# matt-suncy/symbols-from-video

Measured on AMD Instinct MI355X. Metric: frames/sec (enc+binarise+dec fwd+bwd), batch 256x256, 1/2/4/8 MI355X, higher is better.
Workload: dtype bf16; 1 GPU; percep_RBVAE fused train step (batch gather from the HBM-resident latent table + fwd+bwd+losses+Adam), item [16,2,8,4,32,32] per GPU = 256 frames/step/GPU (latents of 256x256 frames), latent 32, 4-layer LSTMs, dropout on; parallelism=dp1, graph=True, dist_world_size=1, schedule=one HIP graph per step, devices_visible=1, graphs_captured=1, launcher=torch.distributed.run or self-spawned ranks

## Files before the change

include/rbvae_dbg_variants.h:

```cpp
#ifndef RBVAE_DBG_VARIANTS_H
#define RBVAE_DBG_VARIANTS_H
#ifdef __cplusplus
extern "C" {
#endif
int rbvae_dbg_wgrad_gemm_variant(int v);

int rbvae_dbg_deconv_last_variant(int v);

#ifdef __cplusplus
}
#endif
#endif
```

include/rbvae_hip.h:

```cpp
#ifndef RBVAE_HIP_H
#define RBVAE_HIP_H

#include <stddef.h>
#include <stdint.h>

#ifdef __cplusplus
extern "C" {
#endif

#define RBVAE_OK 0
#define RBVAE_E_INVALID (-1)
#define RBVAE_E_LAUNCH (-2)
#define RBVAE_E_UNSUPPORTED (-3)

#define RBVAE_F32 0
#define RBVAE_BF16 1

int rbvae_version(void);
int rbvae_counter_add(unsigned long long* counter, unsigned long long inc, void* stream);
const char* rbvae_last_error(void);

int rbvae_binarize_kl_fwd(const float* h, const float* U, float* y_soft, float* z, float* kl_mean,
                          int rows, int L, float tau, float noise_ratio, float noise_eps, int hard,
                          float kl_p, float kl_eps, int kl_clamp, unsigned long long seed,
// ... 19 lines not shown
                       float* dx1, float* dx2, long dstride1, long dstride2, int accumulate, void* stream);
int rbvae_paircos_fwd(const float* x1, const float* x2, long stride1, long stride2, int rows, int L, int label,
                      float margin, float eps, float* out_mean, void* stream);
int rbvae_paircos_bwd(const float* x1, const float* x2, long stride1, long stride2, int rows, int L, int label,
                      float margin, float eps, float scale, const float* gscale_dev, float* dx1, float* dx2, long dstride1,
                      long dstride2, void* stream);
int rbvae_contrast_term_fwd(const float* h0, const float* h1, int B, int T, int L, float* out, void* stream);
int rbvae_contrast_term_bwd(const float* h0, const float* h1, int B, int T, int L, float scale,
                            const float* gscale_dev, float* dh0, float* dh1, void* stream);
int rbvae_contrast_term_nparts(int B, int T);
int rbvae_contrast_term_fused(const float* h0, const float* h1, int B, int T, int L, float scale,
                              const float* gscale_dev, float* parts, float* dh0, float* dh1, void* stream);
int rbvae_triplet_fwd(const float* a, const float* p, const float* n, long sa, long sp, long sn, int rows, int L,
                      float margin, float eps, int swap, float* out_mean, void* stream);
int rbvae_triplet_bwd(const float* a, const float* p, const float* n, long sa, long sp, long sn, int rows, int L,
                      float margin, float eps, int swap, float scale, const float* gscale_dev,
                      float* da, float* dp, float* dn, long dsa, long dsp, long dsn, int accumulate, void* stream);
int rbvae_triplet_term_fwd(const float* h0, const float* h1, int B, int T, int L, float margin, float* out,
                           void* stream);
int rbvae_triplet_term_bwd(const float* h0, const float* h1, int B, int T, int L, float margin, float scale,
                           const float* gscale_dev, float* dh0, float* dh1, void* stream);

size_t rbvae_mse_ws_floats(long n);
int rbvae_mse_fwd(const float* a, const float* b, long n, float* out_mean, float* ws, void* stream);
int rbvae_mse_bwd(const float* a, const float* b, long n, float scale, const float* gscale_dev, float* da,
                  void* stream);

int rbvae_gather_gemm(int dtype, const void* A, const void* W, void* Out, const float* bias, const void* gate,
                      const void* mask, const void* addend, const void* zero_page, int Nimg, int IH, int IW, int TH, int TW, int sa,
                      int OH, int OW, int so, int Kc, int Nout, int lda, int ldo, int taps_total, int nclass,
                      const int* class_desc, int relu, int drop_mode, float drop_p, float scale,
                      unsigned long long seed, const unsigned long long* seed_dev, float* colsum_ws,
                      void* stream);

int rbvae_conv3x3s2_halo_ok(int dtype, int Nimg, int IH, int IW, int Kc, int Nout);
int rbvae_conv3x3s2_halo_colsum_rows(int Nimg, int IH, int IW);
int rbvae_conv3x3s2_halo(int dtype, const void* A, const void* W, void* Out, const float* bias, const void* gate, const void* mask,
                         int Nimg, int IH, int IW, int Kc, int Nout, int lda, int ldo, int relu, int drop_mode, float drop_p,
                         float scale, unsigned long long seed, const unsigned long long* seed_dev, float* colsum_ws, void* stream);

int rbvae_fc_gemm_ok(int dtype, int M, int K, int N, int lda, int ldo);
int rbvae_fc_gemm(int dtype, const void* A, const void* W, void* Out, const float* bias, float* colsum_ws, int M, int K,
                  int N, int lda, int ldo, void* stream);

int rbvae_conv_gather_index(int* idx, int Nimg, int IH, int IW, int OH, int OW, int KH, int KW, int stride,
                            int pad, void* stream);
int rbvae_wgrad_gemm(int dtype, const void* Dy, const void* In, float* dW_slabs, const int* idx,
                     const void* zero_page, int P, int in_rows, int Co, int Ci, int ldy, int ldi, int taps, int ksplit,
                     void* stream);

int rbvae_wgrad3x3s2_halo_ok(int dtype, int Nimg, int OH, int OW, int Ca, int Cb);
int rbvae_wgrad3x3s2_halo_blocks(int Nimg, int OH, int OW);
int rbvae_wgrad3x3s2_halo(int dtype, const void* S, const void* G, float* dW_slabs, const void* zero_page, int Nimg, int OH,
                          int OW, int Ca, int Cb, int lds, int ldg, int ksplit, void* stream);

int rbvae_wgrad3x3s2_row_ok(int dtype, int Nimg, int OH, int OW, int Ca, int Cb);
int rbvae_wgrad3x3s2_row_blocks(int Nimg, int OH, int OW);
int rbvae_wgrad3x3s2_row(int dtype, const void* S, const void* G, float* dW_slabs, const void* zero_page, int Nimg, int OH,
                         int OW, int Ca, int Cb, int lds, int ldg, int ksplit, void* stream);

int rbvae_pack3(int dtype, const float* in, void* out, int d0, int d1, int d2, long s0, long s1, long s2,
                void* stream);
int rbvae_permute_reduce(const float* in, int nslab, long slab_stride, float* out, int d0, int d1, int d2, long s0,
                         long s1, long s2, float scale, int accumulate, void* stream);
int rbvae_cast_pad(int dtype, const float* in, void* out, int rows, int L, int Lpad, void* stream);
int rbvae_reduce_rows(const float* ws, int rows, int C, float* out, float scale, int accumulate, void* stream);
// ... 365 lines not shown
```

symbols-from-video_amd/build.py:

```python
import concurrent.futures
import os
import subprocess
import sys

HERE = os.path.dirname(os.path.abspath(__file__))
CSRC = os.path.join(HERE, "csrc")
OBJ = os.path.join(HERE, "build")
LIB = os.path.join(HERE, "librbvae_hip.so")
DBG_LIB = os.path.join(HERE, "librbvae_dbg.so")
DEBUG_LIB = os.path.join(HERE, "librbvae_hip_debug.so")
DBG_SOURCES = ("dbg.hip",)
HIPCC = os.environ.get("HIPCC", "/opt/rocm/bin/hipcc")
FLAGS = ["--offload-arch=gfx950", "-O3", "-fPIC", "-std=c++17", "-Wall", "-Wno-unused-function"]


def sources():
    return sorted(f for f in os.listdir(CSRC) if f.endswith(".hip"))


def _stale(target, deps):
    if not os.path.exists(target):
        return True
    t = os.path.getmtime(target)
    return any(os.path.getmtime(d) > t for d in deps)


def _compile(src, extra=(), suffix=""):
    obj = os.path.join(OBJ, src[:-4] + suffix + ".o")
    headers = [os.path.join(CSRC, f) for f in os.listdir(CSRC) if f.endswith(".h")]
    headers.append(os.path.join(os.path.dirname(HERE), "include", "rbvae_hip.h"))
    if _stale(obj, [os.path.join(CSRC, src)] + headers):
        cmd = [HIPCC] + FLAGS + list(extra) + ["-c", os.path.join(CSRC, src), "-o", obj]
        r = subprocess.run(cmd, capture_output=True, text=True)
        if r.returncode != 0:
            raise RuntimeError(f"hipcc failed on {src}:\n{r.stdout}\n{r.stderr}")
        if src in ISA_CHECKED and not extra:
            try:
                _check_asm_reads(src)
            except Exception:
                os.remove(obj)
                raise
        return obj, True
    return obj, False


ISA_CHECKED = {
    "wgrad_gemm.hip": ("_ZN5rbvae12wgrad_gemm_k", ("ds_read_b64_tr_b16",)),
    "gather_gemm.hip": ("_ZN5rbvae13gather_gemm_k", ("ds_read_b128",)),
    "conv_halo.hip": ("_ZN5rbvae11conv_halo_k", ("ds_read_b128",)),
    "conv_halo_ws.hip": ("_ZN5rbvae14conv_halo_ws_k", ("ds_read_b128",)),
    "deconv_halo.hip": ("_ZN5rbvae13deconv_halo_k", ("ds_read_b128",)),
    "wgrad_halo.hip": ("_ZN5rbvae12wgrad_halo_k", ("ds_read_b64_tr_b16",)),
    "wgrad_row.hip": ("_ZN5rbvae11wgrad_row_k", ("ds_read_b64_tr_b16",)),
    "conv_s2.hip": ("_ZN5rbvae9conv_s2_k", ("ds_read_b128",)),
    "upconv.hip": ("_ZN5rbvae13upconv_halo_k", ("ds_read_b128",)),
    "conv_first.hip": (("_ZN5rbvae13wgrad_first_k", "_ZN5rbvae18wgrad_first_wide_k"), ("ds_read_b64_tr_b16",)),
    "deconv_last_bwd.hip": ("_ZN5rbvae21deconv_last_fwd_bwd_k", ("ds_read_b128",)),
}


ASM_VMEM_LOADS = {"conv_halo.hip": "global_load_dwordx4", "deconv_halo.hip": "global_load_dwordx4",
                  "conv_halo_ws.hip": "buffer_load_dwordx4", "upconv.hip": "global_load_dwordx4"}


def _check_asm_reads(src):
    import importlib.util
    spec = importlib.util.spec_from_file_location("rbvae_isa_check", os.path.join(HERE, "isa_check.py"))
    mod = importlib.util.module_from_spec(spec)
    spec.loader.exec_module(mod)
    asm = os.path.join(OBJ, src[:-4] + ".s")
    cmd = [HIPCC] + FLAGS + ["-S", "--cuda-device-only", os.path.join(CSRC, src), "-o", asm]
    r = subprocess.run(cmd, capture_output=True, text=True)
    if r.returncode != 0:
        raise RuntimeError(f"hipcc -S failed on {src}:\n{r.stderr}")
    prefixes, ops = ISA_CHECKED[src]
    bad = []
    for prefix in ((prefixes,) if isinstance(prefixes, str) else prefixes):
        bad += mod.tr_asm_hazards(open(asm).read(), prefix, ops)
        if src in ASM_VMEM_LOADS:
            bad += mod.asm_vmem_load_hazards(open(asm).read(), prefix, ASM_VMEM_LOADS[src])
    if bad:
        raise RuntimeError(src + " ISA check failed (fragment register touched before its wait):\n" + "\n".join(bad[:20]))


def build(verbose=False):
    os.makedirs(OBJ, exist_ok=True)
    with concurrent.futures.ThreadPoolExecutor(max_workers=min(8, os.cpu_count() or 2)) as ex:
        res = list(ex.map(_compile, sources()))
    objs = [o for (o, _), src in zip(res, sources()) if src not in DBG_SOURCES]
    dbg_objs = [o for (o, _), src in zip(res, sources()) if src in DBG_SOURCES]

    def link(target, objects, extra=()):
        if _stale(target, objects) or any(c for _, c in res):
            cmd = [HIPCC, "--offload-arch=gfx950", "-shared", "-fPIC", "-o", target] + objects + list(extra)
            r = subprocess.run(cmd, capture_output=True, text=True)
            if r.returncode != 0:
                raise RuntimeError(f"link failed:\n{r.stdout}\n{r.stderr}")
            if verbose:
                print("built", target)

    link(LIB, objs)
    link(DBG_LIB, dbg_objs, ["-L" + HERE, "-lrbvae_hip", "-Wl,-rpath,$ORIGIN"])
    if os.environ.get("RBVAE_DEBUG") == "1":
        stamped = ["-DGG_STAMPS=1", "-DWG_STAMPS=1"]
        with concurrent.futures.ThreadPoolExecutor(max_workers=min(8, os.cpu_count() or 2)) as ex:
            dres = list(ex.map(lambda s_: _compile(s_, stamped, ".dbg"), [s_ for s_ in sources() if s_ not in DBG_SOURCES]))
        link(DEBUG_LIB, [o for o, _ in dres])
    return LIB


if __name__ == "__main__":
    build(verbose=True)
    sys.exit(0)
# ... 1 lines not shown
```

symbols-from-video_amd/csrc/dbg.hip:

```cpp
#include "mma.h"

namespace rbvae {

__global__ void dbg_mfma_bf16_k(const bf16_t* A, const bf16_t* B, float* D) {
    const int l = threadIdx.x, m = l & 15, g = l >> 4;
    bf16x8_t a, b;
    for (int j = 0; j < 8; ++j) {
        a[j] = (short)A[m * 32 + 8 * g + j];
        b[j] = (short)B[(8 * g + j) * 16 + m];
    }
    f32x4_t acc = {0.f, 0.f, 0.f, 0.f};
    acc = __builtin_amdgcn_mfma_f32_16x16x32_bf16(a, b, acc, 0, 0, 0);
    for (int r = 0; r < 4; ++r) D[(4 * g + r) * 16 + m] = acc[r];
}
__global__ void dbg_mfma_f32_k(const float* A, const float* B, float* D) {
    const int l = threadIdx.x, m = l & 15, g = l >> 4;
    f32x4_t acc = {0.f, 0.f, 0.f, 0.f};
    acc = __builtin_amdgcn_mfma_f32_16x16x4f32(A[m * 4 + g], B[g * 16 + m], acc, 0, 0, 0);
    for (int r = 0; r < 4; ++r) D[(4 * g + r) * 16 + m] = acc[r];
}
__global__ void dbg_glds_k(const unsigned* src, const int* lane_src_chunk, unsigned* out) {
    __shared__ __attribute__((aligned(16))) unsigned lds[256];
    const int l = threadIdx.x;
    glds16(src + 4 * lane_src_chunk[l], lds);
// ... 35 lines not shown
                       (bf16_t*)out);
    RBVAE_CHECK_LAUNCH("dbg_tr16");
    return RBVAE_OK;
}
}

namespace rbvae { extern int ch_variant; }
extern "C" int rbvae_dbg_conv_halo_variant(int v) {
    const int old = rbvae::ch_variant;
    rbvae::ch_variant = v;
    return old;
}

namespace rbvae { extern int lstm_unit_threads; }
extern "C" int rbvae_dbg_lstm_unit_threads(int v) {
    const int old = rbvae::lstm_unit_threads;
    rbvae::lstm_unit_threads = v;
    return old;
}

namespace rbvae { extern int wgrad_gemm_variant; }
extern "C" int rbvae_dbg_wgrad_gemm_variant(int v) {
    const int old = rbvae::wgrad_gemm_variant;
    rbvae::wgrad_gemm_variant = v;
    return old;
}

namespace rbvae { extern int deconv_last_variant; }
extern "C" int rbvae_dbg_deconv_last_variant(int v) {
    const int old = rbvae::deconv_last_variant;
    rbvae::deconv_last_variant = v;
    return old;
}
```

symbols-from-video_amd/csrc/gather_gemm.hip:

```cpp
#include "epilogue.h"
#include <stdlib.h>
#include <type_traits>

namespace rbvae {

struct TapClass {
    int ntaps;
    int oh0, ow0;
    signed char widx[16];
    signed char dh[16], dw[16];
};

struct GgArgs {
    const unsigned char* A;
    const unsigned char* W;
    unsigned char* Out;
    const float* bias;
    const unsigned char* gate;
    const unsigned char* mask;
    const unsigned char* addend;
    const unsigned char* zero;
    int Nimg, IH, IW;
    int TH, TW;
    int sa;
// ... 266 lines not shown
        int cbuf = 0;
        read_half(lds0, 0, fa0, fb0);
        const bool late = WAVES == 8 && w >= 4 && p.dephase;
        for (int s = 0; s + 1 < nsteps; ++s) {
            const unsigned lcur = lds0 + cbuf * STAGE;
            cbuf = (cbuf + 1 == GG_NS) ? 0 : cbuf + 1;
            read_half(lcur, 1, fa1, fb1);
            landed(Younger{}, fa0, fb0);
            __builtin_amdgcn_sched_barrier(0);
            mma_half(fa0, fb0);
            __builtin_amdgcn_sched_barrier(0);
            landed(None{}, fa1, fb1);
            if (GG_NS > 2 && nsteps - s - 2 >= GG_NS - 2) wait_vm_lgkm_barrier<(GG_NS > 2 ? GG_NS - 2 : 0) * LOADS>();
            else wait_vm_lgkm_barrier<0>();
            if (!late && s + GG_NS < nsteps) stage_next();
            read_half(lds0 + cbuf * STAGE, 0, fa0, fb0);
            __builtin_amdgcn_sched_barrier(0);
            mma_half(fa1, fb1);
            __builtin_amdgcn_sched_barrier(0);
            if (late && s + GG_NS < nsteps) stage_next();
        }
        {
            const unsigned lcur = lds0 + cbuf * STAGE;
            read_half(lcur, 1, fa1, fb1);
            landed(Younger{}, fa0, fb0);
            __builtin_amdgcn_sched_barrier(0);
            mma_half(fa0, fb0);
            __builtin_amdgcn_sched_barrier(0);
            landed(None{}, fa1, fb1);
            __builtin_amdgcn_sched_barrier(0);
            mma_half(fa1, fb1);
        }
    }
    GG_STAMP(3);
    __syncthreads();

    constexpr int CPR = BN / EC;
    constexpr int RL = THREADS / CPR;
    constexpr int ITERS = BM / RL;
    constexpr bool PREFETCH = GG_PREFETCH && ITERS <= 8;
    constexpr bool PF_LATE = GG_PREFETCH == 2;
    const int sch = tid % CPR, rl = tid / CPR;
    const int scol = n0 + sch * EC;
    int orow_[ITERS];
    u32x4_t gv[PREFETCH ? ITERS : 1], av[PREFETCH ? ITERS : 1];
#pragma unroll
    for (int it = 0; it < ITERS; ++it) {
        const int o = s_orow[it * RL + rl];
        orow_[it] = scol < p.Nout ? o : -1;
        if constexpr (PREFETCH && !PF_LATE) {
            const size_t off = ((size_t)(orow_[it] < 0 ? 0 : orow_[it]) * p.ldo + (orow_[it] < 0 ? 0 : scol)) * ES;
            if (p.gate) gv[it] = *(const u32x4_t*)(p.gate + off);
            if (p.addend) av[it] = *(const u32x4_t*)(p.addend + off);
        }
    }

    unsigned char* tile = smem;
#pragma unroll
    for (int nt = 0; nt < NTW; ++nt) {
        const int cb = (wc * NTW + nt) * 16 + 4 * fg;
#if GG_BIAS_LDS
        const float4 b4 = *(const float4*)(s_bias + cb);
        const float bz[4] = {b4.x, b4.y, b4.z, b4.w};
#else
        float bz[4] = {0.f, 0.f, 0.f, 0.f};
        if (p.bias && n0 + cb < p.Nout) {
            const float4 b4 = *(const float4*)(p.bias + n0 + cb);
            bz[0] = b4.x; bz[1] = b4.y; bz[2] = b4.z; bz[3] = b4.w;
        }
        (void)s_bias;
#endif
#pragma unroll
        for (int mt = 0; mt < MT; ++mt) {
            const int row = (wr * MT + mt) * 16 + fi;
            float v[4];
#pragma unroll
            for (int r = 0; r < 4; ++r) v[r] = epi_act(acc[mt][nt][r], bz[r], p.relu, p.scale);
            epi_stage<T>(tile + row * PITCH + cb * ES, v[0], v[1], v[2], v[3]);
        }
    }
    if constexpr (PREFETCH && PF_LATE) {
        if (p.gate) {
#pragma unroll
            for (int it = 0; it < ITERS; ++it) {
                const size_t off = ((size_t)(orow_[it] < 0 ? 0 : orow_[it]) * p.ldo + (orow_[it] < 0 ? 0 : scol)) * ES;
                gv[it] = *(const u32x4_t*)(p.gate + off);
            }
        }
    }
    __syncthreads();
    GG_STAMP(4);

    float csum[EC];
#pragma unroll
    for (int e = 0; e < EC; ++e) csum[e] = 0.f;
    DropKey dkey{0u, 0u};
    if (p.drop_mode == 1) dkey = epi_drop_key(p.seed, p.seed_dev);
#pragma unroll
    for (int it = 0; it < ITERS; ++it) {
        const int row = it * RL + rl;
        const int orow = orow_[it];
        if (orow >= 0) {
            const int col = scol;
            u32x4_t val = *(const u32x4_t*)(tile + row * PITCH + sch * 16);
            T* ev = (T*)&val;
            if (p.drop_mode == 1) {
                const unsigned run = drop_run(dkey, (unsigned long long)orow * p.Nout + col);
                if constexpr (sizeof(T) == 2) drop_chunk_zero_b16<EC>(run, p.drop_thresh >> 16, (unsigned*)&val);
                else drop_chunk_zero_f32<EC>(run, p.drop_thresh >> 16, (float*)&val);
            } else if (p.drop_mode == 2) {
                const unsigned char* mk = p.mask + (size_t)orow * p.Nout + col;
#pragma unroll
                for (int e = 0; e < EC; ++e)
                    if (!mk[e]) ev[e] = 0;
            }
            if (p.addend) {
                u32x4_t a4;
                if constexpr (PREFETCH && !PF_LATE) a4 = av[it];
                else a4 = *(const u32x4_t*)(p.addend + ((size_t)orow * p.ldo + col) * ES);
                const T* ae = (const T*)&a4;
#pragma unroll
                for (int e = 0; e < EC; ++e) Elem<T>::store(ev + e, Elem<T>::load(ev + e) + Elem<T>::load(ae + e));
            }
            if (p.gate) {
                u32x4_t g4;
                if constexpr (PREFETCH) g4 = gv[it];
                else g4 = *(const u32x4_t*)(p.gate + ((size_t)orow * p.ldo + col) * ES);
#pragma unroll
                for (int e = 0; e < EC; ++e)
                    if (!elem_pos<T>((const unsigned char*)&g4, e)) ev[e] = 0;
            }
            *(u32x4_t*)(p.Out + ((size_t)orow * p.ldo + col) * ES) = val;
            if (p.colsum_ws) {
#pragma unroll
                for (int e = 0; e < EC; ++e) csum[e] += Elem<T>::load(ev + e);
            }
        }
    }
    GG_STAMP(5);
    if (p.colsum_ws) {
        lds_barrier();
        float* red = (float*)smem;
#pragma unroll
        for (int e = 0; e < EC; ++e) red[rl * BN + sch * EC + e] = csum[e];
        lds_barrier();
        if (tid < BN && n0 + tid < p.Nout) {
            float t = 0.f;
#pragma unroll
            for (int k = 0; k < RL; ++k) t += red[k * BN + tid];
            p.colsum_ws[((size_t)bz * gridDim.x + bx) * p.Nout + n0 + tid] = t;
        }
    }
#if GG_STAMPS
    if (p.stamps) {
        asm volatile("s_waitcnt vmcnt(0)" ::: "memory");
        GG_STAMP(6);
    }
#endif
}

template <typename T, int NT, int WAVES, int NS, int OCC = 1, int BM = GG_BM>
static int launch_gg(const GgArgs& a, hipStream_t st) {
    constexpr int BN = NT * 32;
    constexpr int ES = sizeof(T);
    const int Mc = a.Nimg * a.TH * a.TW;
    const size_t ring = (size_t)NS * (BM * 128 + BN * 128);
    const size_t tile = (size_t)BM * (BN * ES + 16);
    const size_t lds = (ring > tile ? ring : tile) + BM * sizeof(int) + 64 * sizeof(int) + BN * sizeof(float);
    static bool attr_set = false;
    if (!attr_set) {
        hipFuncSetAttribute((const void*)gather_gemm_k<T, NT, WAVES, NS, OCC, BM>, hipFuncAttributeMaxDynamicSharedMemorySize,
                            (int)lds);
        attr_set = true;
    }
    dim3 grid(cdiv(Mc, BM), cdiv(a.Nout, BN), a.nclass);
    hipLaunchKernelGGL((gather_gemm_k<T, NT, WAVES, NS, OCC, BM>), grid, dim3(WAVES * 64), lds, st, a);
    RBVAE_CHECK_LAUNCH("gather_gemm");
    return RBVAE_OK;
}

#ifndef GG_RING64
#define GG_RING64 6
#endif
#ifndef GG_WAVES64
#define GG_WAVES64 4
#endif

template <typename T>
static int dispatch_gg(const GgArgs& a, hipStream_t st, int max_steps) {
    const long blocks = (long)cdiv(a.Nimg * a.TH * a.TW, GG_BM) * cdiv(a.Nout, a.Nout > 64 ? 128 : 64) * a.nclass;
    constexpr int force = 0;
    constexpr int dbg = 0;
    int ns = max_steps <= 2 ? 1 : (blocks > 256 ? 2 : 3);
    if (force) ns = force;
    if (ns == 3 && blocks > 128 && max_steps >= 8) ns = 4;
    if (a.Nout <= 64 && blocks <= 128 && max_steps >= 16 && sizeof(T) == 2 && !a.colsum_ws && !a.xcd_order)
        return launch_gg<T, 2, GG_WAVES64, GG_RING64, 1, 64>(a, st);
    if (a.Nout <= 64) return ns == 1 ? launch_gg<T, 2, 4, 1>(a, st) : launch_gg<T, 2, 4, 2>(a, st);
    constexpr int small = 2;
    if (ns == 3 && !force && !dbg && small) {
        constexpr int sq = 1;
        if (sq && small >= 2 && blocks <= 64 && !a.colsum_ws && !a.xcd_order && sizeof(T) == 2)
            return launch_gg<T, 2, GG_WAVES64, GG_RING64, 1, 64>(a, st);
        if (small >= 2 && blocks <= 64) return launch_gg<T, 1, 4, 3>(a, st);
        if (blocks <= 128) return launch_gg<T, 2, 4, 3>(a, st);
    }
    constexpr int one = 1;
    if (ns == 1 && one >= 1 && blocks > 512) return launch_gg<T, 2, 4, 1, 4>(a, st);
    if (ns == 1 && one >= 2 && blocks <= 64) return launch_gg<T, 1, 4, 1>(a, st);
    if (ns == 1) return launch_gg<T, 4, 4, 1>(a, st);
    if (ns >= 2 && (dbg == 5 || dbg == 6)) return dbg == 5 ? launch_gg<T, 2, 4, 3>(a, st) : launch_gg<T, 2, 4, 2>(a, st);
    if (ns == 2) return launch_gg<T, 4, 8, 2>(a, st);
    if (dbg == 4) return launch_gg<T, 4, 4, 3>(a, st);
    if (ns >= 4) return launch_gg<T, 4, 8, 4>(a, st);
    return launch_gg<T, 4, 8, 3>(a, st);
}

}

using namespace rbvae;

static unsigned long long* g_gg_stamps = nullptr;
#if GG_STAMPS
extern "C" int rbvae_dbg_gg_stamps(unsigned long long* buf, void* stream) {
    (void)stream;
    g_gg_stamps = buf;
    return RBVAE_OK;
}
#endif

extern "C" int rbvae_gather_gemm(int dtype, const void* A, const void* W, void* Out, const float* bias,
                                 const void* gate, const void* mask, const void* addend, const void* zero_page, int Nimg, int IH,
                                 int IW, int TH, int TW, int sa, int OH, int OW, int so, int Kc, int Nout, int lda,
                                 int ldo, int taps_total, int nclass, const int* class_desc, int relu,
                                 int drop_mode, float drop_p, float scale, unsigned long long seed,
                                 const unsigned long long* seed_dev, float* colsum_ws, void* stream) {
    RBVAE_CHECK_ARG(A && W && Out && zero_page && class_desc, "gather_gemm: null pointer");
    RBVAE_CHECK_ARG(dtype == RBVAE_F32 || dtype == RBVAE_BF16, "gather_gemm: dtype %d", dtype);
    const int ES = dtype == RBVAE_F32 ? 4 : 2;
    const int KE = 128 / ES;
    RBVAE_CHECK_ARG(Kc > 0 && Kc % KE == 0, "gather_gemm: Kc=%d must be a multiple of %d", Kc, KE);
    RBVAE_CHECK_ARG(Nout > 0 && Nout % 8 == 0, "gather_gemm: Nout=%d must be a multiple of 8", Nout);
    RBVAE_CHECK_ARG(lda >= Kc && (lda * ES) % 16 == 0 && ldo >= Nout && (ldo * ES) % 16 == 0,
                    "gather_gemm: leading dimensions lda=%d ldo=%d", lda, ldo);
    RBVAE_CHECK_ARG(nclass >= 1 && nclass <= 4, "gather_gemm: nclass=%d", nclass);
    RBVAE_CHECK_ARG(Nimg > 0 && IH > 0 && IW > 0 && TH > 0 && TW > 0 && OH > 0 && OW > 0, "gather_gemm: bad grid");
// ... 4 lines not shown
    GgArgs a;
    if (const int e = epi_drop_args("gather_gemm", drop_mode, mask, drop_p, &a.drop_thresh)) return e;
    a.A = (const unsigned char*)A; a.W = (const unsigned char*)W; a.Out = (unsigned char*)Out; a.bias = bias;
    a.gate = (const unsigned char*)gate; a.mask = (const unsigned char*)mask; a.addend = (const unsigned char*)addend;
    a.zero = (const unsigned char*)zero_page;
    a.Nimg = Nimg; a.IH = IH; a.IW = IW; a.TH = TH; a.TW = TW; a.sa = sa; a.OH = OH; a.OW = OW; a.so = so;
    a.Kc = Kc; a.Nout = Nout; a.lda = lda; a.ldo = ldo; a.taps_total = taps_total;
    a.relu = relu; a.drop_mode = drop_mode; a.scale = scale; a.seed = seed; a.seed_dev = seed_dev; a.colsum_ws = colsum_ws;
    a.nclass = nclass;
    constexpr int dephase = 1;
    a.dephase = dephase;
    constexpr int xcd = 0;
    a.xcd_order = xcd && cdiv(Nimg * TH * TW, GG_BM) % 8 == 0 && (nclass > 1 || cdiv(Nout, Nout > 64 ? 128 : 64) > 1);
    a.stamps = g_gg_stamps;
    auto log2_or_neg = [](int v) { int s = 0; while ((1 << s) < v) ++s; return (1 << s) == v ? s : -1; };
    a.sh_thw = log2_or_neg(TH * TW);
    a.sh_tw = log2_or_neg(TW);
    const int* d = class_desc;
    for (int c = 0; c < nclass; ++c) {
        TapClass& t = a.cls[c];
        t.ntaps = d[0]; t.oh0 = d[1]; t.ow0 = d[2];
        RBVAE_CHECK_ARG(t.ntaps >= 1 && t.ntaps <= 16, "gather_gemm: class %d has %d taps", c, t.ntaps);
        d += 3;
        for (int j = 0; j < t.ntaps; ++j) {
            RBVAE_CHECK_ARG(d[0] >= 0 && d[0] < taps_total, "gather_gemm: tap index %d outside [0,%d)", d[0], taps_total);
            t.widx[j] = (signed char)d[0]; t.dh[j] = (signed char)d[1]; t.dw[j] = (signed char)d[2];
            d += 3;
        }
    }
    hipStream_t st = (hipStream_t)stream;
    int max_taps = 0;
    for (int c = 0; c < nclass; ++c) max_taps = a.cls[c].ntaps > max_taps ? a.cls[c].ntaps : max_taps;
    const int max_steps = max_taps * (Kc / KE);
    return dtype == RBVAE_F32 ? dispatch_gg<float>(a, st, max_steps) : dispatch_gg<bf16_t>(a, st, max_steps);
}
```

Before: 588,700 frames/s.

## Add patch-reuse gather GEMM kernel for stride-2 3x3 convs sharing A tiles across taps

Adds a new gather_patch_k kernel for bf16 stride-2 single-class tap sets. Taps are grouped by input parity plane, so one staged A tile is reused across taps whose offsets differ only by a row or column shift. The host builds a precomputed step plan of weight offsets, ring slots and fresh-load flags, and the kernel reads it via readlane. This cuts redundant global-to-LDS A loads. The cost is more complex addressing, edge masking for shifted rows, and new dispatch paths for the 64-row and 128-row tile cases. The epilogue is factored into a shared header, and a debug switch, a plan-query API and an ISA check are added.

```diff
diff --git a/include/rbvae_dbg_variants.h b/include/rbvae_dbg_variants.h
--- a/include/rbvae_dbg_variants.h
+++ b/include/rbvae_dbg_variants.h
@@ -7,6 +7,8 @@
 
 int rbvae_dbg_deconv_last_variant(int v);
 
+int rbvae_dbg_gather_patch_variant(int v);
+
 #ifdef __cplusplus
 }
 #endif
diff --git a/include/rbvae_hip.h b/include/rbvae_hip.h
--- a/include/rbvae_hip.h
+++ b/include/rbvae_hip.h
@@ -75,6 +75,7 @@
                       const int* class_desc, int relu, int drop_mode, float drop_p, float scale,
                       unsigned long long seed, const unsigned long long* seed_dev, float* colsum_ws,
                       void* stream);
+int rbvae_gather_patch_plan(int sa, int so, int nclass, int ntaps, const int* taps, int Kc, int* steps, int max_steps);
 
 int rbvae_conv3x3s2_halo_ok(int dtype, int Nimg, int IH, int IW, int Kc, int Nout);
 int rbvae_conv3x3s2_halo_colsum_rows(int Nimg, int IH, int IW);
diff --git a/symbols-from-video_amd/build.py b/symbols-from-video_amd/build.py
--- a/symbols-from-video_amd/build.py
+++ b/symbols-from-video_amd/build.py
@@ -1,5 +1,6 @@
 import concurrent.futures
 import os
+import re
 import subprocess
 import sys
 
@@ -59,6 +60,11 @@
 }
 
 
+ISA_CHECKED_ALSO = {
+    "gather_gemm.hip": ("_ZN5rbvae14gather_patch_k", ("ds_read_b128",)),
+}
+
+
 ASM_VMEM_LOADS = {"conv_halo.hip": "global_load_dwordx4", "deconv_halo.hip": "global_load_dwordx4",
                   "conv_halo_ws.hip": "buffer_load_dwordx4", "upconv.hip": "global_load_dwordx4"}
 
@@ -79,6 +85,12 @@
         bad += mod.tr_asm_hazards(open(asm).read(), prefix, ops)
         if src in ASM_VMEM_LOADS:
             bad += mod.asm_vmem_load_hazards(open(asm).read(), prefix, ASM_VMEM_LOADS[src])
+    if src in ISA_CHECKED_ALSO:
+        prefix, ops = ISA_CHECKED_ALSO[src]
+        found = mod.tr_asm_hazards(open(asm).read(), prefix, ops)
+        if not re.search(r"^" + prefix + r"\w+:", open(asm).read(), re.M):
+            found = [prefix + ": no such kernel in the listing"]
+        bad += found
     if bad:
         raise RuntimeError(src + " ISA check failed (fragment register touched before its wait):\n" + "\n".join(bad[:20]))
 
diff --git a/symbols-from-video_amd/csrc/dbg.hip b/symbols-from-video_amd/csrc/dbg.hip
--- a/symbols-from-video_amd/csrc/dbg.hip
+++ b/symbols-from-video_amd/csrc/dbg.hip
@@ -91,3 +91,10 @@
     rbvae::deconv_last_variant = v;
     return old;
 }
+
+namespace rbvae { extern int gather_patch_variant; }
+extern "C" int rbvae_dbg_gather_patch_variant(int v) {
+    const int old = rbvae::gather_patch_variant;
+    rbvae::gather_patch_variant = v;
+    return old;
+}
diff --git a/symbols-from-video_amd/csrc/gather_gemm.hip b/symbols-from-video_amd/csrc/gather_gemm.hip
--- a/symbols-from-video_amd/csrc/gather_gemm.hip
+++ b/symbols-from-video_amd/csrc/gather_gemm.hip
@@ -322,131 +322,353 @@
             mma_half(fa1, fb1);
         }
     }
-    GG_STAMP(3);
+#include "gather_gemm_store.h"
+}
+
+constexpr int GP_MAX_STEPS = 64;
+struct PatchPlan {
+    int ntaps, nplanes;
+    unsigned long long widx;
+    unsigned long long tap;
+    unsigned shift;
+    unsigned plane;
+    unsigned end;
+};
+
+struct PatchArgs {
+    GgArgs g;
+    int nsteps;
+    unsigned stepP[GP_MAX_STEPS];
+    unsigned stepA[GP_MAX_STEPS];
+    unsigned stepC[GP_MAX_STEPS];
+};
+
+struct PlanWalk {
+    int pi, q0, q1, q, kc;
+    __host__ __device__ __forceinline__ void start(const PatchPlan& pl) {
+        pi = 0; q0 = 0; q1 = (int)(pl.end & 15u); q = 0; kc = 0;
+    }
+    __host__ __device__ __forceinline__ bool fresh() const { return q == q0; }
+    __host__ __device__ __forceinline__ void next(const PatchPlan& pl, int kchunks) {
+        if (++q == q1) {
+            if (++kc == kchunks) {
+                kc = 0; ++pi; q0 = q1;
+                q1 = (int)((pl.end >> (4 * pi)) & 15u);
+            }
+            q = q0;
+        }
+    }
+};
+
+static bool patch_plan_build(const TapClass& tc, int taps_total, PatchPlan* pl) {
+    if (tc.ntaps < 1 || tc.ntaps > 9 || taps_total > 128 || tc.oh0 != 0 || tc.ow0 != 0) return false;
+    unsigned seen = 0;
+    for (int j = 0; j < tc.ntaps; ++j) {
+        const int dh = tc.dh[j], dw = tc.dw[j];
+        if (dh < -1 || dh > 1 || dw < -1 || dw > 1) return false;
+        const unsigned bit = 1u << ((dh + 1) * 3 + dw + 1);
+        if (seen & bit) return false;
+        seen |= bit;
+    }
+    *pl = PatchPlan{tc.ntaps, 0, 0ull, 0ull, 0u, 0u, 0u};
+    int q = 0;
+    for (int plane = 3; plane >= 0; --plane) {
+        const int q_first = q;
+        for (int j = 0; j < tc.ntaps; ++j) {
+            const int dh = tc.dh[j], dw = tc.dw[j];
+            if ((((dh & 1) << 1) | (dw & 1)) != plane) continue;
+            pl->widx |= (unsigned long long)tc.widx[j] << (7 * q);
+            pl->tap |= (unsigned long long)j << (4 * q);
+            pl->shift |= (unsigned)((dh < 0 ? 1 : 0) | (dw < 0 ? 2 : 0)) << (2 * q);
+            ++q;
+        }
+        if (q == q_first) continue;
+        pl->plane |= (unsigned)plane << (2 * pl->nplanes);
+        pl->end |= (unsigned)q << (4 * pl->nplanes);
+        ++pl->nplanes;
+    }
+    return true;
+}
+
+static bool patch_steps_fit(const GgArgs& a, int ntaps) {
+    return ntaps * (a.Kc / 64) <= GP_MAX_STEPS && (size_t)a.taps_total * a.Kc * 2 < (1u << 24) &&
+           ((size_t)(a.IW + 1) * a.lda + a.Kc) * 2 < (1ull << 32);
+}
+static void patch_steps_build(const PatchPlan& pl, const GgArgs& a, int NS, PatchArgs* pa) {
+    const int kchunks = a.Kc / 64, nsteps = pl.ntaps * kchunks;
+    pa->nsteps = nsteps;
+    bool fresh[GP_MAX_STEPS + 8] = {};
+    PlanWalk wk;
+    wk.start(pl);
+    int unit = -1;
+    for (int t = 0; t < GP_MAX_STEPS; ++t) {
+        pa->stepP[t] = pa->stepA[t] = pa->stepC[t] = 0u;
+        if (t >= nsteps) continue;
+        fresh[t] = wk.fresh();
+        unit += fresh[t] ? 1 : 0;
+        const unsigned widx = (unsigned)((pl.widx >> (7 * wk.q)) & 127u), plane = (pl.plane >> (2 * wk.pi)) & 3u;
+        const unsigned sh = (pl.shift >> (2 * wk.q)) & 3u;
+        const unsigned aslot = (unsigned)(unit % NS);
+        pa->stepP[t] = (widx * (unsigned)a.Kc + (unsigned)wk.kc * 64u) * 2u | (unsigned)(t % NS) << 24 | aslot << 28 |
+                       (fresh[t] ? 1u << 31 : 0u);
+        pa->stepA[t] = (unsigned)((((size_t)(plane >> 1) * a.IW + (plane & 1)) * a.lda + (size_t)wk.kc * 64) * 2);
+        pa->stepC[t] = ((sh & 1u) * (unsigned)a.TW + (sh >> 1)) | (sh & 1u) << 8 | (sh >> 1) << 9 | aslot << 16;
+        wk.next(pl, kchunks);
+    }
+    for (int t = 0; t < nsteps; ++t) {
+        unsigned nf = 0;
+        for (int k = t + 1; k <= t + NS - 2; ++k) nf += fresh[k] ? 1u : 0u;
+        pa->stepC[t] |= nf << 12;
+    }
+}
+
+template <int NT, int WAVES, int NS, int BM>
+__global__ __launch_bounds__(WAVES * 64, 1) void gather_patch_k(const PatchArgs pa) {
+    using T = bf16_t;
+    const GgArgs& p = pa.g;
+    constexpr int THREADS = WAVES * 64;
+    static_assert(BM % 32 == 0 && BM + 32 <= THREADS && NS >= 3, "tile rows / ring depth");
+    constexpr int BN = NT * 32;
+    constexpr int ES = sizeof(T);
+    constexpr int EC = 16 / ES;
+    constexpr int A_BYTES = BM * 128, B_BYTES = BN * 128;
+    constexpr int W_OFF = NS * A_BYTES;
+    constexpr int PITCH = BN * ES + 16;
+    constexpr int WR = 2, WC = WAVES / 2;
+    constexpr int MT = (BM / 16) / WR, NTW = (2 * NT) / WC;
+    constexpr int A_INSTR = (BM / 8) / WAVES, B_INSTR = (BN / 8) / WAVES;
+    static_assert(NTW >= 1 && B_INSTR >= 1 && A_INSTR >= 1 && MT >= 1, "tile too small for this many waves");
+    static_assert((NS - 2) * (A_INSTR + B_INSTR) <= 63, "vmcnt is a 6-bit counter");
+    constexpr int RING = NS * (A_BYTES + B_BYTES) > BM * PITCH ? NS * (A_BYTES + B_BYTES) : BM * PITCH;
+    extern __shared__ __attribute__((aligned(16))) unsigned char smem[];
+    unsigned* s_zero = (unsigned*)(smem + RING);
+    int* s_orow = (int*)(smem + RING + 128);
+    float* s_bias = (float*)(s_orow + BM);
+
+    const int tid = threadIdx.x, lane = tid & 63;
+    const int w = __builtin_amdgcn_readfirstlane(tid >> 6);
+    GG_STAMP(0);
+    const unsigned bx = blockIdx.x, by = blockIdx.y, bz = blockIdx.z;
+    const int Mc = p.Nimg * p.TH * p.TW;
+    const int m0 = bx * BM, n0 = by * BN;
+
+#if GG_BIAS_LDS
+    for (int i = tid; i < BN; i += THREADS) s_bias[i] = (p.bias && n0 + i < p.Nout) ? p.bias[n0 + i] : 0.f;
+#endif
+    if (tid < BM) {
+        const int m = m0 + tid;
+        s_orow[tid] = m < Mc ? m : -1;
+    } else if (tid < BM + 32) {
+        s_zero[tid - BM] = 0u;
+    }
     __syncthreads();
-
-    constexpr int CPR = BN / EC;
-    constexpr int RL = THREADS / CPR;
-    constexpr int ITERS = BM / RL;
-    constexpr bool PREFETCH = GG_PREFETCH && ITERS <= 8;
-    constexpr bool PF_LATE = GG_PREFETCH == 2;
-    const int sch = tid % CPR, rl = tid / CPR;
-    const int scol = n0 + sch * EC;
-    int orow_[ITERS];
-    u32x4_t gv[PREFETCH ? ITERS : 1], av[PREFETCH ? ITERS : 1];
-#pragma unroll
-    for (int it = 0; it < ITERS; ++it) {
-        const int o = s_orow[it * RL + rl];
-        orow_[it] = scol < p.Nout ? o : -1;
-        if constexpr (PREFETCH && !PF_LATE) {
-            const size_t off = ((size_t)(orow_[it] < 0 ? 0 : orow_[it]) * p.ldo + (orow_[it] < 0 ? 0 : scol)) * ES;
-            if (p.gate) gv[it] = *(const u32x4_t*)(p.gate + off);
-            if (p.addend) av[it] = *(const u32x4_t*)(p.addend + off);
-        }
-    }
-
-    unsigned char* tile = smem;
-#pragma unroll
-    for (int nt = 0; nt < NTW; ++nt) {
-        const int cb = (wc * NTW + nt) * 16 + 4 * fg;
-#if GG_BIAS_LDS
-        const float4 b4 = *(const float4*)(s_bias + cb);
-        const float bz[4] = {b4.x, b4.y, b4.z, b4.w};
-#else
-        float bz[4] = {0.f, 0.f, 0.f, 0.f};
-        if (p.bias && n0 + cb < p.Nout) {
-            const float4 b4 = *(const float4*)(p.bias + n0 + cb);
-            bz[0] = b4.x; bz[1] = b4.y; bz[2] = b4.z; bz[3] = b4.w;
-        }
-        (void)s_bias;
-#endif
+    GG_STAMP(1);
+
+    const int srow = lane >> 3, schunk = lane & 7;
+    const unsigned char* abase[A_INSTR];
+    bool aval[A_INSTR];
+#pragma unroll
+    for (int i = 0; i < A_INSTR; ++i) {
+        const int u = (w * A_INSTR + i) * 8 + srow;
+        const int m = m0 + u;
+        aval[i] = m < Mc;
+        int n = 0, r = 0, c = 0;
+        if (aval[i]) split_row(p, m, n, r, c);
+        abase[i] = aval[i] ? p.A + ((size_t)((n * p.IH + 2 * r) * p.IW + 2 * c) * p.lda) * ES + (schunk ^ ((u >> 1) & 7)) * 16
+                           : p.zero + schunk * 16;
+    }
+    const unsigned char* bptr[B_INSTR];
+    bool bval[B_INSTR];
+#pragma unroll
+    for (int i = 0; i < B_INSTR; ++i) {
+        const int r = (w * B_INSTR + i) * 8 + srow;
+        const int n = n0 + r;
+        bval[i] = n < p.Nout;
+        bptr[i] = bval[i] ? p.W + ((size_t)n * p.taps_total * p.Kc) * ES + (schunk ^ ((r >> 1) & 7)) * 16 : p.zero + schunk * 16;
+    }
+
+    const int nsteps = pa.nsteps;
+    const unsigned vP = pa.stepP[lane], vA = pa.stepA[lane], vC = pa.stepC[lane];
+
+    int pt = 0;
+    const unsigned char* bsrc[B_INSTR];
+    const unsigned char* asrc[A_INSTR];
+    unsigned lb_off = 0, la_off = 0, pfresh = 0;
+    auto stage_prepare = [&]() {
+        const unsigned rP = (unsigned)__builtin_amdgcn_readlane((int)vP, pt);
+        const unsigned rA = (unsigned)__builtin_amdgcn_readlane((int)vA, pt);
+        const unsigned woff = rP & 0xffffffu;
+        pfresh = rP >> 31;
+        lb_off = W_OFF + ((rP >> 24) & 15u) * B_BYTES + (w * B_INSTR) * 1024;
+        la_off = ((rP >> 28) & 7u) * A_BYTES + (w * A_INSTR) * 1024;
+#pragma unroll
+        for (int i = 0; i < B_INSTR; ++i) {
+            bsrc[i] = bptr[i] + (bval[i] ? woff : 0u);
+            asm volatile("" : "+v"(bsrc[i]));
+        }
+        if (pfresh) {
+#pragma unroll
+            for (int i = 0; i < A_INSTR; ++i) {
+                asrc[i] = abase[i] + (aval[i] ? rA : 0u);
+                asm volatile("" : "+v"(asrc[i]));
+            }
+        }
+        ++pt;
+    };
+    auto stage_issue = [&]() {
+#pragma unroll
+        for (int i = 0; i < B_INSTR; ++i) glds16(bsrc[i], smem + lb_off + i * 1024);
+        if (pfresh) {
+#pragma unroll
+            for (int i = 0; i < A_INSTR; ++i) glds16(asrc[i], smem + la_off + i * 1024);
+        }
+    };
+    auto stage_next = [&]() { stage_prepare(); stage_issue(); };
+    int nfresh = 0;
+    auto wait_stage_barrier = [&]() {
+        static_for<0, NS - 1>([&](auto I) {
+            constexpr int NF = decltype(I)::value;
+            if (nfresh == NF) wait_vm_lgkm_barrier<(NS - 2) * B_INSTR + NF * A_INSTR>();
+        });
+    };
+
+    const int fi = lane & 15, fg = lane >> 4;
+    const int fsw = (fi >> 1) & 7;
+    const int wr = w / WC, wc = w - wr * WC;
+    int offB[2];
+#pragma unroll
+    for (int kk = 0; kk < 2; ++kk) offB[kk] = W_OFF + (wc * NTW * 16 + fi) * 128 + (((4 * kk + fg) ^ fsw) * 16);
+    unsigned top = 0, left = 0;
+#pragma unroll
+    for (int mt = 0; mt < MT; ++mt) {
+        const int row = (wr * MT + mt) * 16 + fi;
+        const int rem = row & ((1 << p.sh_thw) - 1);
+        top |= (unsigned)((rem >> p.sh_tw) == 0) << mt;
+        left |= (unsigned)((rem & ((1 << p.sh_tw) - 1)) == 0) << mt;
+    }
+    const unsigned lds0 = (unsigned)(size_t)(__attribute__((address_space(3))) unsigned char*)smem;
+    const unsigned zaddr = lds0 + RING + fg * 16;
+    unsigned aad[MT];
+    auto step_addresses = [&](int step) {
+        const unsigned rC = (unsigned)__builtin_amdgcn_readlane((int)vC, step);
+        nfresh = (int)((rC >> 12) & 15u);
+        const int row0 = wr * MT * 16 + fi - (int)(rC & 255u);
+        const unsigned a0 = lds0 + ((rC >> 16) & 15u) * A_BYTES + (unsigned)(row0 * 128) + (unsigned)(((fg ^ (row0 >> 1)) & 7) * 16);
+        const unsigned out = ((rC & 256u) ? top : 0u) | ((rC & 512u) ? left : 0u);
 #pragma unroll
         for (int mt = 0; mt < MT; ++mt) {
-            const int row = (wr * MT + mt) * 16 + fi;
-            float v[4];
-#pragma unroll
-            for (int r = 0; r < 4; ++r) v[r] = epi_act(acc[mt][nt][r], bz[r], p.relu, p.scale);
-            epi_stage<T>(tile + row * PITCH + cb * ES, v[0], v[1], v[2], v[3]);
-        }
-    }
-    if constexpr (PREFETCH && PF_LATE) {
-        if (p.gate) {
-#pragma unroll
-            for (int it = 0; it < ITERS; ++it) {
-                const size_t off = ((size_t)(orow_[it] < 0 ? 0 : orow_[it]) * p.ldo + (orow_[it] < 0 ? 0 : scol)) * ES;
-                gv[it] = *(const u32x4_t*)(p.gate + off);
-            }
-        }
-    }
-    __syncthreads();
-    GG_STAMP(4);
-
-    float csum[EC];
-#pragma unroll
-    for (int e = 0; e < EC; ++e) csum[e] = 0.f;
-    DropKey dkey{0u, 0u};
-    if (p.drop_mode == 1) dkey = epi_drop_key(p.seed, p.seed_dev);
-#pragma unroll
-    for (int it = 0; it < ITERS; ++it) {
-        const int row = it * RL + rl;
-        const int orow = orow_[it];
-        if (orow >= 0) {
-            const int col = scol;
-            u32x4_t val = *(const u32x4_t*)(tile + row * PITCH + sch * 16);
-            T* ev = (T*)&val;
-            if (p.drop_mode == 1) {
-                const unsigned run = drop_run(dkey, (unsigned long long)orow * p.Nout + col);
-                if constexpr (sizeof(T) == 2) drop_chunk_zero_b16<EC>(run, p.drop_thresh >> 16, (unsigned*)&val);
-                else drop_chunk_zero_f32<EC>(run, p.drop_thresh >> 16, (float*)&val);
-            } else if (p.drop_mode == 2) {
-                const unsigned char* mk = p.mask + (size_t)orow * p.Nout + col;
-#pragma unroll
-                for (int e = 0; e < EC; ++e)
-                    if (!mk[e]) ev[e] = 0;
-            }
-            if (p.addend) {
-                u32x4_t a4;
-                if constexpr (PREFETCH && !PF_LATE) a4 = av[it];
-                else a4 = *(const u32x4_t*)(p.addend + ((size_t)orow * p.ldo + col) * ES);
-                const T* ae = (const T*)&a4;
-#pragma unroll
-                for (int e = 0; e < EC; ++e) Elem<T>::store(ev + e, Elem<T>::load(ev + e) + Elem<T>::load(ae + e));
-            }
-            if (p.gate) {
-                u32x4_t g4;
-                if constexpr (PREFETCH) g4 = gv[it];
-                else g4 = *(const u32x4_t*)(p.gate + ((size_t)orow * p.ldo + col) * ES);
-#pragma unroll
-                for (int e = 0; e < EC; ++e)
-                    if (!elem_pos<T>((const unsigned char*)&g4, e)) ev[e] = 0;
-            }
-            *(u32x4_t*)(p.Out + ((size_t)orow * p.ldo + col) * ES) = val;
-            if (p.colsum_ws) {
-#pragma unroll
-                for (int e = 0; e < EC; ++e) csum[e] += Elem<T>::load(ev + e);
-            }
-        }
-    }
-    GG_STAMP(5);
-    if (p.colsum_ws) {
-        lds_barrier();
-        float* red = (float*)smem;
-#pragma unroll
-        for (int e = 0; e < EC; ++e) red[rl * BN + sch * EC + e] = csum[e];
-        lds_barrier();
-        if (tid < BN && n0 + tid < p.Nout) {
-            float t = 0.f;
-#pragma unroll
-            for (int k = 0; k < RL; ++k) t += red[k * BN + tid];
-            p.colsum_ws[((size_t)bz * gridDim.x + bx) * p.Nout + n0 + tid] = t;
-        }
-    }
-#if GG_STAMPS
-    if (p.stamps) {
-        asm volatile("s_waitcnt vmcnt(0)" ::: "memory");
-        GG_STAMP(6);
-    }
-#endif
+            aad[mt] = ((out >> mt) & 1u) ? zaddr : a0 + mt * 2048;
+            asm volatile("" : "+v"(aad[mt]));
+        }
+    };
+
+    f32x4_t acc[MT][NTW];
+#pragma unroll
+    for (int mt = 0; mt < MT; ++mt)
+#pragma unroll
+        for (int nt = 0; nt < NTW; ++nt) acc[mt][nt] = f32x4_t{0.f, 0.f, 0.f, 0.f};
+
+    constexpr int RPH = MT + NTW;
+    static_assert(RPH <= 15, "lgkmcnt is a 4-bit counter");
+    auto read_half = [&](unsigned wbase, int kk, u32x4_t (&fa)[MT], u32x4_t (&fb)[NTW]) {
+        const unsigned ab_ = wbase + offB[kk];
+#pragma unroll
+        for (int mt = 0; mt < MT; ++mt) {
+            const unsigned aa_ = aad[mt] ^ (unsigned)(kk * 64);
+            asm volatile("ds_read_b128 %0, %1" : "=v"(fa[mt]) : "v"(aa_));
+        }
+#pragma unroll
+        for (int nt = 0; nt < NTW; ++nt)
+            asm volatile("ds_read_b128 %0, %1 offset:%2" : "=v"(fb[nt]) : "v"(ab_), "n"(nt * 2048));
+    };
+    auto landed = [&](auto younger_tag, u32x4_t (&fa)[MT], u32x4_t (&fb)[NTW]) {
+        constexpr int YOUNGER = decltype(younger_tag)::value;
+        static_assert((MT == 4 || MT == 2) && NTW == 2, "operand list below");
+        if constexpr (MT == 2)
+            asm volatile("s_waitcnt lgkmcnt(%4)" : "+v"(fa[0]), "+v"(fa[MT - 1]), "+v"(fb[0]), "+v"(fb[1]) : "n"(YOUNGER));
+        else
+            asm volatile("s_waitcnt lgkmcnt(%6)"
+                         : "+v"(fa[0]), "+v"(fa[1]), "+v"(fa[2 % MT]), "+v"(fa[3 % MT]), "+v"(fb[0]), "+v"(fb[1])
+                         : "n"(YOUNGER));
+    };
+    auto mma_half = [&](const u32x4_t (&fa)[MT], const u32x4_t (&fb)[NTW]) {
+#pragma unroll
+        for (int mt = 0; mt < MT; ++mt)
+#pragma unroll
+            for (int nt = 0; nt < NTW; ++nt) Mma<T>::run(acc[mt][nt], fb[nt], fa[mt]);
+    };
+    using Younger = std::integral_constant<int, RPH>;
+    using None = std::integral_constant<int, 0>;
+    u32x4_t fa0[MT], fb0[NTW], fa1[MT], fb1[NTW];
+    GG_STAMP(2);
+    {
+#pragma unroll
+        for (int i = 0; i < NS - 1; ++i)
+            if (i < nsteps) stage_next();
+        nfresh = (int)(((unsigned)__builtin_amdgcn_readlane((int)vC, 0) >> 12) & 15u);
+        if (nsteps > NS - 1) wait_stage_barrier();
+        else wait_vm_lgkm_barrier<0>();
+        if (NS - 1 < nsteps) stage_next();
+        int cbuf = 0;
+        step_addresses(0);
+        read_half(lds0, 0, fa0, fb0);
+        const bool late = WAVES == 8 && w >= 4 && p.dephase;
+        for (int s = 0; s + 1 < nsteps; ++s) {
+            const unsigned lcur = lds0 + cbuf * B_BYTES;
+            cbuf = (cbuf + 1 == NS) ? 0 : cbuf + 1;
+            read_half(lcur, 1, fa1, fb1);
+            landed(Younger{}, fa0, fb0);
+            __builtin_amdgcn_sched_barrier(0);
+            mma_half(fa0, fb0);
+            __builtin_amdgcn_sched_barrier(0);
+            step_addresses(s + 1);
+            const bool more = s + NS < nsteps;
+            if (more) stage_prepare();
+            __builtin_amdgcn_sched_barrier(0);
+            landed(None{}, fa1, fb1);
+            if (s + NS - 1 < nsteps) wait_stage_barrier();
+            else wait_vm_lgkm_barrier<0>();
+            if (!late && more) stage_issue();
+            read_half(lds0 + cbuf * B_BYTES, 0, fa0, fb0);
+            __builtin_amdgcn_sched_barrier(0);
+            mma_half(fa1, fb1);
+            __builtin_amdgcn_sched_barrier(0);
+            if (late && more) stage_issue();
+        }
+        {
+            const unsigned lcur = lds0 + cbuf * B_BYTES;
+            read_half(lcur, 1, fa1, fb1);
+            landed(Younger{}, fa0, fb0);
+            __builtin_amdgcn_sched_barrier(0);
+            mma_half(fa0, fb0);
+            __builtin_amdgcn_sched_barrier(0);
+            landed(None{}, fa1, fb1);
+            __builtin_amdgcn_sched_barrier(0);
+            mma_half(fa1, fb1);
+        }
+    }
+#include "gather_gemm_store.h"
+}
+
+template <int NT, int WAVES, int NS, int BM>
+static int launch_gp(const GgArgs& a, const PatchPlan& pl, hipStream_t st) {
+    constexpr int BN = NT * 32;
+    const int Mc = a.Nimg * a.TH * a.TW;
+    const size_t ring = (size_t)NS * (BM * 128 + BN * 128);
+    const size_t tile = (size_t)BM * (BN * 2 + 16);
+    const size_t lds = (ring > tile ? ring : tile) + 128 + BM * sizeof(int) + BN * sizeof(float);
+    static bool attr_set = false;
+    if (!attr_set) {
+        hipFuncSetAttribute((const void*)gather_patch_k<NT, WAVES, NS, BM>, hipFuncAttributeMaxDynamicSharedMemorySize, (int)lds);
+        attr_set = true;
+    }
+    PatchArgs pa;
+    pa.g = a;
+    patch_steps_build(pl, a, NS, &pa);
+    dim3 grid(cdiv(Mc, BM), cdiv(a.Nout, BN), 1);
+    hipLaunchKernelGGL((gather_patch_k<NT, WAVES, NS, BM>), grid, dim3(WAVES * 64), lds, st, pa);
+    RBVAE_CHECK_LAUNCH("gather_gemm (patch planes)");
+    return RBVAE_OK;
 }
 
 template <typename T, int NT, int WAVES, int NS, int OCC = 1, int BM = GG_BM>
@@ -476,22 +698,52 @@
 #define GG_WAVES64 4
 #endif
 
+#ifndef GP_VARIANT_DEFAULT
+#define GP_VARIANT_DEFAULT 0
+#endif
+int gather_patch_variant = GP_VARIANT_DEFAULT;
+
+constexpr int GP_NS128 = 4, GP_NS64 = GG_RING64;
+#ifndef GP_PRODUCT128
+#define GP_PRODUCT128 0
+#endif
+#ifndef GP_PRODUCT64
+#define GP_PRODUCT64 0
+#endif
+
+static int patch_tile_rows(const GgArgs& a) {
+    if (a.nclass != 1 || a.sa != 2 || a.so != 1 || a.IH != 2 * a.TH || a.IW != 2 * a.TW || a.OH != a.TH || a.OW != a.TW) return 0;
+    if (a.Kc % 64 != 0 || a.xcd_order) return 0;
+    const int thw = a.TH * a.TW;
+    return thw == 64 ? 128 : (thw == 16 && !a.colsum_ws ? 64 : 0);
+}
+
 template <typename T>
-static int dispatch_gg(const GgArgs& a, hipStream_t st, int max_steps) {
+static int dispatch_gg(const GgArgs& a, hipStream_t st, int max_steps, const PatchPlan* pl = nullptr) {
+    if constexpr (sizeof(T) == 2) {
+        if (pl && gather_patch_variant == 2 && patch_tile_rows(a) == 128) return launch_gp<4, 8, GP_NS128, 128>(a, *pl, st);
+        if (pl && gather_patch_variant == 3 && patch_tile_rows(a) == 64) return launch_gp<2, GG_WAVES64, GP_NS64, 64>(a, *pl, st);
+    }
+    const bool patch128 = sizeof(T) == 2 && pl && gather_patch_variant == 0 && GP_PRODUCT128 && patch_tile_rows(a) == 128;
+    const bool patch64 = sizeof(T) == 2 && pl && gather_patch_variant == 0 && GP_PRODUCT64 && patch_tile_rows(a) == 64;
     const long blocks = (long)cdiv(a.Nimg * a.TH * a.TW, GG_BM) * cdiv(a.Nout, a.Nout > 64 ? 128 : 64) * a.nclass;
     constexpr int force = 0;
     constexpr int dbg = 0;
     int ns = max_steps <= 2 ? 1 : (blocks > 256 ? 2 : 3);
     if (force) ns = force;
     if (ns == 3 && blocks > 128 && max_steps >= 8) ns = 4;
-    if (a.Nout <= 64 && blocks <= 128 && max_steps >= 16 && sizeof(T) == 2 && !a.colsum_ws && !a.xcd_order)
+    if (a.Nout <= 64 && blocks <= 128 && max_steps >= 16 && sizeof(T) == 2 && !a.colsum_ws && !a.xcd_order) {
+        if (patch64) return launch_gp<2, GG_WAVES64, GP_NS64, 64>(a, *pl, st);
         return launch_gg<T, 2, GG_WAVES64, GG_RING64, 1, 64>(a, st);
+    }
     if (a.Nout <= 64) return ns == 1 ? launch_gg<T, 2, 4, 1>(a, st) : launch_gg<T, 2, 4, 2>(a, st);
     constexpr int small = 2;
     if (ns == 3 && !force && !dbg && small) {
         constexpr int sq = 1;
-        if (sq && small >= 2 && blocks <= 64 && !a.colsum_ws && !a.xcd_order && sizeof(T) == 2)
+        if (sq && small >= 2 && blocks <= 64 && !a.colsum_ws && !a.xcd_order && sizeof(T) == 2) {
+            if (patch64) return launch_gp<2, GG_WAVES64, GP_NS64, 64>(a, *pl, st);
             return launch_gg<T, 2, GG_WAVES64, GG_RING64, 1, 64>(a, st);
+        }
         if (small >= 2 && blocks <= 64) return launch_gg<T, 1, 4, 3>(a, st);
         if (blocks <= 128) return launch_gg<T, 2, 4, 3>(a, st);
     }
@@ -502,6 +754,7 @@
     if (ns >= 2 && (dbg == 5 || dbg == 6)) return dbg == 5 ? launch_gg<T, 2, 4, 3>(a, st) : launch_gg<T, 2, 4, 2>(a, st);
     if (ns == 2) return launch_gg<T, 4, 8, 2>(a, st);
     if (dbg == 4) return launch_gg<T, 4, 4, 3>(a, st);
+    if (patch128) return launch_gp<4, 8, GP_NS128, 128>(a, *pl, st);
     if (ns >= 4) return launch_gg<T, 4, 8, 4>(a, st);
     return launch_gg<T, 4, 8, 3>(a, st);
 }
@@ -572,5 +825,43 @@
     int max_taps = 0;
     for (int c = 0; c < nclass; ++c) max_taps = a.cls[c].ntaps > max_taps ? a.cls[c].ntaps : max_taps;
     const int max_steps = max_taps * (Kc / KE);
-    return dtype == RBVAE_F32 ? dispatch_gg<float>(a, st, max_steps) : dispatch_gg<bf16_t>(a, st, max_steps);
-}
+    if (dtype == RBVAE_F32) return dispatch_gg<float>(a, st, max_steps);
+    PatchPlan plan;
+    const bool patch = gather_patch_variant != 1 && patch_tile_rows(a) && patch_plan_build(a.cls[0], taps_total, &plan) &&
+                       patch_steps_fit(a, a.cls[0].ntaps);
+    return dispatch_gg<bf16_t>(a, st, max_steps, patch ? &plan : nullptr);
+}
+
+extern "C" int rbvae_gather_patch_plan(int sa, int so, int nclass, int ntaps, const int* taps, int Kc, int* steps,
+                                       int max_steps) {
+    RBVAE_CHECK_ARG(taps && ntaps >= 1 && max_steps >= 0 && (steps || max_steps == 0), "gather_patch_plan: arguments");
+    if (sa != 2 || so != 1 || nclass != 1 || ntaps > 9 || Kc <= 0 || Kc % 64 != 0) return RBVAE_E_UNSUPPORTED;
+    TapClass tc;
+    tc.ntaps = ntaps; tc.oh0 = 0; tc.ow0 = 0;
+    int taps_total = 1;
+    for (int j = 0; j < ntaps; ++j) {
+        if (taps[3 * j] < 0 || taps[3 * j] > 127 || taps[3 * j + 1] < -128 || taps[3 * j + 1] > 127 || taps[3 * j + 2] < -128 ||
+            taps[3 * j + 2] > 127)
+            return RBVAE_E_UNSUPPORTED;
+        tc.widx[j] = (signed char)taps[3 * j]; tc.dh[j] = (signed char)taps[3 * j + 1]; tc.dw[j] = (signed char)taps[3 * j + 2];
+        taps_total = taps[3 * j] + 1 > taps_total ? taps[3 * j] + 1 : taps_total;
+    }
+    PatchPlan pl;
+    if (!patch_plan_build(tc, taps_total, &pl)) return RBVAE_E_UNSUPPORTED;
+    const int kchunks = Kc / 64, nsteps = ntaps * kchunks;
+    PlanWalk wk;
+    wk.start(pl);
+    for (int s = 0; s < nsteps && s < max_steps; ++s) {
+        const unsigned sh = (pl.shift >> (2 * wk.q)) & 3u;
+        int* o = steps + 7 * s;
+        o[0] = (int)((pl.plane >> (2 * wk.pi)) & 3u);
+        o[1] = wk.kc;
+        o[2] = (int)((pl.tap >> (4 * wk.q)) & 15u);
+        o[3] = wk.fresh() ? 1 : 0;
+        o[4] = (int)((pl.widx >> (7 * wk.q)) & 127u);
+        o[5] = (sh & 1u) ? -1 : 0;
+        o[6] = (sh & 2u) ? -1 : 0;
+        wk.next(pl, kchunks);
+    }
+    return nsteps;
+}
diff --git a/symbols-from-video_amd/csrc/gather_gemm_store.h b/symbols-from-video_amd/csrc/gather_gemm_store.h
--- /dev/null
+++ b/symbols-from-video_amd/csrc/gather_gemm_store.h
@@ -0,0 +1,125 @@
+    GG_STAMP(3);
+    __syncthreads();
+
+    constexpr int CPR = BN / EC;
+    constexpr int RL = THREADS / CPR;
+    constexpr int ITERS = BM / RL;
+    constexpr bool PREFETCH = GG_PREFETCH && ITERS <= 8;
+    constexpr bool PF_LATE = GG_PREFETCH == 2;
+    const int sch = tid % CPR, rl = tid / CPR;
+    const int scol = n0 + sch * EC;
+    int orow_[ITERS];
+    u32x4_t gv[PREFETCH ? ITERS : 1], av[PREFETCH ? ITERS : 1];
+#pragma unroll
+    for (int it = 0; it < ITERS; ++it) {
+        const int o = s_orow[it * RL + rl];
+        orow_[it] = scol < p.Nout ? o : -1;
+        if constexpr (PREFETCH && !PF_LATE) {
+            const size_t off = ((size_t)(orow_[it] < 0 ? 0 : orow_[it]) * p.ldo + (orow_[it] < 0 ? 0 : scol)) * ES;
+            if (p.gate) gv[it] = *(const u32x4_t*)(p.gate + off);
+            if (p.addend) av[it] = *(const u32x4_t*)(p.addend + off);
+        }
+    }
+
+    unsigned char* tile = smem;
+#pragma unroll
+    for (int nt = 0; nt < NTW; ++nt) {
+        const int cb = (wc * NTW + nt) * 16 + 4 * fg;
+#if GG_BIAS_LDS
+        const float4 b4 = *(const float4*)(s_bias + cb);
+        const float bz[4] = {b4.x, b4.y, b4.z, b4.w};
+#else
+        float bz[4] = {0.f, 0.f, 0.f, 0.f};
+        if (p.bias && n0 + cb < p.Nout) {
+            const float4 b4 = *(const float4*)(p.bias + n0 + cb);
+            bz[0] = b4.x; bz[1] = b4.y; bz[2] = b4.z; bz[3] = b4.w;
+        }
+        (void)s_bias;
+#endif
+#pragma unroll
+        for (int mt = 0; mt < MT; ++mt) {
+            const int row = (wr * MT + mt) * 16 + fi;
+            float v[4];
+#pragma unroll
+            for (int r = 0; r < 4; ++r) v[r] = epi_act(acc[mt][nt][r], bz[r], p.relu, p.scale);
+            epi_stage<T>(tile + row * PITCH + cb * ES, v[0], v[1], v[2], v[3]);
+        }
+    }
+    if constexpr (PREFETCH && PF_LATE) {
+        if (p.gate) {
+#pragma unroll
+            for (int it = 0; it < ITERS; ++it) {
+                const size_t off = ((size_t)(orow_[it] < 0 ? 0 : orow_[it]) * p.ldo + (orow_[it] < 0 ? 0 : scol)) * ES;
+                gv[it] = *(const u32x4_t*)(p.gate + off);
+            }
+        }
+    }
+    __syncthreads();
+    GG_STAMP(4);
+
+    float csum[EC];
+#pragma unroll
+    for (int e = 0; e < EC; ++e) csum[e] = 0.f;
+    DropKey dkey{0u, 0u};
+    if (p.drop_mode == 1) dkey = epi_drop_key(p.seed, p.seed_dev);
+#pragma unroll
+    for (int it = 0; it < ITERS; ++it) {
+        const int row = it * RL + rl;
+        const int orow = orow_[it];
+        if (orow >= 0) {
+            const int col = scol;
+            u32x4_t val = *(const u32x4_t*)(tile + row * PITCH + sch * 16);
+            T* ev = (T*)&val;
+            if (p.drop_mode == 1) {
+                const unsigned run = drop_run(dkey, (unsigned long long)orow * p.Nout + col);
+                if constexpr (sizeof(T) == 2) drop_chunk_zero_b16<EC>(run, p.drop_thresh >> 16, (unsigned*)&val);
+                else drop_chunk_zero_f32<EC>(run, p.drop_thresh >> 16, (float*)&val);
+            } else if (p.drop_mode == 2) {
+                const unsigned char* mk = p.mask + (size_t)orow * p.Nout + col;
+#pragma unroll
+                for (int e = 0; e < EC; ++e)
+                    if (!mk[e]) ev[e] = 0;
+            }
+            if (p.addend) {
+                u32x4_t a4;
+                if constexpr (PREFETCH && !PF_LATE) a4 = av[it];
+                else a4 = *(const u32x4_t*)(p.addend + ((size_t)orow * p.ldo + col) * ES);
+                const T* ae = (const T*)&a4;
+#pragma unroll
+                for (int e = 0; e < EC; ++e) Elem<T>::store(ev + e, Elem<T>::load(ev + e) + Elem<T>::load(ae + e));
+            }
+            if (p.gate) {
+                u32x4_t g4;
+                if constexpr (PREFETCH) g4 = gv[it];
+                else g4 = *(const u32x4_t*)(p.gate + ((size_t)orow * p.ldo + col) * ES);
+#pragma unroll
+                for (int e = 0; e < EC; ++e)
+                    if (!elem_pos<T>((const unsigned char*)&g4, e)) ev[e] = 0;
+            }
+            *(u32x4_t*)(p.Out + ((size_t)orow * p.ldo + col) * ES) = val;
+            if (p.colsum_ws) {
+#pragma unroll
+                for (int e = 0; e < EC; ++e) csum[e] += Elem<T>::load(ev + e);
+            }
+        }
+    }
+    GG_STAMP(5);
+    if (p.colsum_ws) {
+        lds_barrier();
+        float* red = (float*)smem;
+#pragma unroll
+        for (int e = 0; e < EC; ++e) red[rl * BN + sch * EC + e] = csum[e];
+        lds_barrier();
+        if (tid < BN && n0 + tid < p.Nout) {
+            float t = 0.f;
+#pragma unroll
+            for (int k = 0; k < RL; ++k) t += red[k * BN + tid];
+            p.colsum_ws[((size_t)bz * gridDim.x + bx) * p.Nout + n0 + tid] = t;
+        }
+    }
+#if GG_STAMPS
+    if (p.stamps) {
+        asm volatile("s_waitcnt vmcnt(0)" ::: "memory");
+        GG_STAMP(6);
+    }
+#endif
```

Measured after the change: 587,900 frames/s. About the same (-0.1%).
